# jczarnowski/DeepFactors

Measured on NVIDIA B200. Metric: keyframe-pair Jacobian+JtJ evals/sec (640x480, C=32), higher is better.
Workload: dtype f32

## Files before the change

### deepfactors_b200/csrc/dfk_api.cu

```cuda
#include <cuda_runtime.h>
#include <math.h>
#include <stdint.h>
#include <stdio.h>
#include <stdlib.h>
#include <string.h>

#include <algorithm>
#include <new>
#include <string>
#include <vector>

#include "dfk.h"
#include "dfk_internal.h"

using namespace dfk;

struct DfkContext {
  int device = 0;
  int num_sms = 1;
  int sm_limit = 0;
  cudaStream_t own_stream = nullptr;
  cudaStream_t stream = nullptr;
  std::string err;
  DfkSfmAlignerParams params;
// ... 6 lines not shown
  float* out_host = nullptr;
  float* code_dev = nullptr;
  float* track_dev = nullptr;
  size_t track_cap = 0;
  float* track_host = nullptr;
  size_t track_host_cap = 0;

  float* sparse_dev = nullptr;
  size_t sparse_cap = 0;
  float* sparse_host = nullptr;
  size_t sparse_host_cap = 0;
  SfmItemDev* items_dev = nullptr;
  size_t items_cap = 0;
  float* partials_dev = nullptr;
  size_t partials_cap = 0;
  struct RayTab {
    float fx, fy, u0, v0;
    uint32_t w, h;
    float* dev;
  };
  std::vector<RayTab> ray_cache;
  bool ray_miss = false;
  float* codes_dev = nullptr;
  size_t codes_cap = 0;
  std::vector<float> codes_host;
  float* records_dev = nullptr;
  size_t records_cap = 0;
  float* records_host = nullptr;
  size_t records_host_cap = 0;
  std::vector<SfmItemDev> items_host;
// ... 198 lines not shown
  return m % n == 0 ? 1 : m;
}

template <typename T>
cudaError_t ensure(T** ptr, size_t* cap, size_t need)
{
  if (*cap >= need) return cudaSuccess;
  const size_t old_cap = *cap;
  if (*ptr) cudaFree(*ptr);
  *ptr = nullptr;
  *cap = 0;
  size_t n = std::max(need, old_cap * 2);
  cudaError_t e = cudaMalloc(reinterpret_cast<void**>(ptr), n * sizeof(T));
  if (e == cudaSuccess) *cap = n;
  return e;
}

DfkStatus build_items(DfkHandle h, const DfkSfmWorkItem* items, int n, int code_size, int tile_px, int max_ctas,
                      bool want_ray_tabs, const float* codes_dev, SfmLaunchPlan* plan)
{
  h->ray_miss = false;
  const DfkDenseSfmParams& sp = h->params.sfmparams;
  h->items_host.resize(n);
  uint32_t tile_cursor = 0;
  for (int i = 0; i < n; ++i) {
    const DfkSfmWorkItem& w = items[i];
    SfmItemDev& d = h->items_host[i];
    const uint32_t W = w.img0.width, H = w.img0.height;
    if (W == 0 || H == 0) return fail(h, DFK_ERR_INVALID_ARG, "[SfmAligner::RunStep] empty image");
    if (!img_ok(&w.img0, W, H, 1) || !img_ok(&w.img1, W, H, 1) || !img_ok(&w.dpt0, W, H, 1) ||
// ... 168 lines not shown
                                cudaMemcpyHostToDevice, h->stream),
             "[SfmAligner::RunStep] code upload failed");
  const size_t pfloats = tc ? (size_t)kTcPartialFloats : sfm_partial_floats(code_size);
  DFK_CUDA(h, ensure(&h->items_dev, &h->items_cap, (size_t)n), "[SfmAligner::RunStep] scratch allocation failed");
  DFK_CUDA(h, ensure(&h->partials_dev, &h->partials_cap, (size_t)plan.num_partials * pfloats),
           "[SfmAligner::RunStep] scratch allocation failed");
  DFK_CUDA(h, cudaMemcpyAsync(h->items_dev, h->items_host.data(), sizeof(SfmItemDev) * n, cudaMemcpyHostToDevice,
                              h->stream),
           "[SfmAligner::RunStep] work list upload failed");
  cudaEvent_t ev0 = nullptr, ev1 = nullptr;
  if (h->profiling) {
    DfkStatus ps = profile_events(h, &ev0, &ev1);
    if (ps != DFK_OK) return ps;
  }
  if (tc) {
    DFK_CUDA(h, launch_sfm_tc(h->items_dev, plan, h->ray_miss, h->partials_dev, h->stream, ev0, ev1),
             "[SfmAligner::RunStep] kernel launch failed");
    if (h->ray_miss) h->launches += 1;
  } else if (wide) {
    DFK_CUDA(h, launch_sfm_wide(code_size, h->items_dev, plan, h->partials_dev, h->stream, ev0, ev1),
             "[SfmAligner::RunStep] kernel launch failed");
  } else {
    DFK_CUDA(h, launch_sfm_fp32(code_size, h->items_dev, plan, h->partials_dev, records_dev, h->stream, ev0, ev1),
             "[SfmAligner::RunStep] kernel launch failed");
  }
  DFK_CUDA(h, launch_sfm_finalize(code_size, tc, h->items_dev, n, h->partials_dev, records_dev, h->stream),
           "[SfmAligner::RunStep] kernel launch failed");
  h->launches += 2;
  return DFK_OK;
}

}

extern "C" {

int dfk_version(void) { return DFK_VERSION; }

const char* dfk_status_string(DfkStatus s)
{
  switch (s) {
    case DFK_OK: return "ok";
// ... 47 lines not shown
  } catch (...) {
    return DFK_ERR_NOMEM;
  }
}

DfkStatus dfk_destroy(DfkHandle h)
{
  try {
    if (!h) return DFK_OK;
    DeviceGuard guard(h->device);
    if (h->own_stream) cudaStreamSynchronize(h->own_stream);
    cudaFree(h->simple_scratch); cudaFree(h->counter); cudaFree(h->out_dev); cudaFree(h->code_dev);
    cudaFree(h->track_dev);
    cudaFree(h->codes_dev);
    if (h->track_host) cudaFreeHost(h->track_host);
    cudaFree(h->items_dev); cudaFree(h->partials_dev); cudaFree(h->records_dev);
    for (auto& r : h->ray_cache) cudaFree(r.dev);
    if (h->out_host) cudaFreeHost(h->out_host);
    if (h->records_host) cudaFreeHost(h->records_host);
    for (cudaEvent_t e : h->ev_pool) cudaEventDestroy(e);
    if (h->own_stream) cudaStreamDestroy(h->own_stream);
    delete h;
    return DFK_OK;
  } catch (...) {
    return oom(h);
  }
}

DfkStatus dfk_set_stream(DfkHandle h, void* cuda_stream)
{
  try {
// ... 952 lines not shown
```

### deepfactors_b200/csrc/dfk_internal.h

```cpp
#pragma once

#include <cuda_runtime.h>
#include <stdint.h>

#include <string>
#include <vector>

#include "dfk.h"

namespace dfk {

struct SfmItemDev {
  float q[4];
  float t[3];
  float R[9];
  float fx, fy, u0, v0;
  float border;
  float ulim;
  float vlim;
  float min_dpt, avg_dpt, huber_delta;
  const float* img0;
  const float* img1;
  const float* dpt0;
  float* valid0;
// ... 22 lines not shown
template <int C>
struct SfmCfg {
  static constexpr int NF = C + 7;
  static constexpr int NFP = (NF + 7) & ~7;
  static constexpr int NB = NFP / 8;
  static constexpr int NBLK = NB * (NB + 1) / 2;
  static constexpr int PARTIAL_FLOATS = NFP * NFP + 8;
};

constexpr int kTilePixels = 256;
constexpr int kTcTilePixels = 128;
constexpr int kTcRows = 80;
constexpr int kTcCols = 40;
constexpr int kTcRowsPad = 96;
constexpr int kTcPartialFloats = kTcRowsPad * kTcCols + 8;

struct SfmLaunchPlan {
  int num_items = 0;
  int num_tiles = 0;
  int num_ctas = 0;
  int num_partials = 0;
  int max_ctas_per_item = 0;
};

cudaError_t launch_sfm_fp32(int code_size, const SfmItemDev* items_dev, const SfmLaunchPlan& plan,
                            float* partials_dev, float* records_dev, cudaStream_t stream,
                            cudaEvent_t ev_start = nullptr, cudaEvent_t ev_stop = nullptr);
cudaError_t launch_sfm_finalize(int code_size, bool tc, const SfmItemDev* items_dev, int num_items,
                                const float* partials_dev, float* records_dev, cudaStream_t stream);
constexpr int sfm_wide_tile_pixels(int code_size) { return code_size >= 128 ? 64 : 128; }
bool sfm_wide_supported(int code_size);
cudaError_t launch_sfm_wide(int code_size, const SfmItemDev* items_dev, const SfmLaunchPlan& plan,
                            float* partials_dev, cudaStream_t stream, cudaEvent_t ev_start = nullptr,
                            cudaEvent_t ev_stop = nullptr);
bool sfm_tc_supported(int code_size);
cudaError_t launch_sfm_tc(const SfmItemDev* items_dev, const SfmLaunchPlan& plan, bool build_ray_tables,
                          float* partials_dev, cudaStream_t stream, cudaEvent_t ev_start = nullptr,
                          cudaEvent_t ev_stop = nullptr);
size_t sfm_partial_floats(int code_size);
constexpr int sfm_fp32_ctas_per_sm(int code_size) { return code_size <= 8 ? 2 : 1; }
bool sfm_fp32_supported(int code_size);
int sfm_max_ctas();

struct PixelCam {
  float q[4], t[3];
  float fx, fy, u0, v0, border, ulim, vlim, min_dpt;
};
struct View {
  const float* ptr;
  uint32_t pitch;
};
cudaError_t launch_se3_step(const PixelCam& pc, float huber_delta, int width, int height, View img0, View img1,
                            View dpt0, View grad1, bool grad_aligned, float* scratch, unsigned int* counter,
// ... 52 lines not shown
```

### deepfactors_b200/csrc/dfk_sfm_finalize.cu

```cuda
#include <cuda_runtime.h>
#include <stdint.h>

#include "dfk_internal.h"

namespace dfk {

namespace {

constexpr int kFinWarps = 8;
constexpr int kFinUnroll = 4;

__device__ __forceinline__ int packed_index(int i, int j, int NP) { return i * NP - (i * (i - 1)) / 2 + (j - i); }

__device__ __forceinline__ int tc_hrow(int f) { return f < 32 ? f : 64 + (f - 32); }
__device__ __forceinline__ int tc_lrow(int f) { return f < 32 ? 32 + f : 72 + (f - 32); }

template <int C, bool TC>
__global__ void __launch_bounds__(kFinWarps * 32)
sfm_finalize_kernel(const SfmItemDev* __restrict__ items, const float* __restrict__ partials,
                    float* __restrict__ records)
{
  using Cfg = SfmCfg<C>;
  constexpr int NFP = Cfg::NFP;
  constexpr int NP = 12 + C;
  constexpr int NH = NP * (NP + 1) / 2;
  constexpr int REC = NH + NP + 2;
  constexpr int NE = (C + 7 > 49) ? (C + 7) : 49;
  constexpr int EPL = (NE + 31) / 32;
  constexpr int PSTRIDE = TC ? kTcPartialFloats : Cfg::PARTIAL_FLOATS;
  constexpr int INL_OFF = TC ? kTcRowsPad * kTcCols : NFP * NFP;
  constexpr int NOFF = TC ? 3 : 1;
  __shared__ float red[kFinWarps][EPL * 32];
  __shared__ unsigned int red_inl[kFinWarps];
  __shared__ float sum[EPL * 32];

  cudaGridDependencySynchronize();
  const SfmItemDev& I = items[blockIdx.x];
  const int unit = blockIdx.y;
  const int warp = threadIdx.x >> 5, lane = threadIdx.x & 31;
  const float* P = partials + (size_t)I.partial_begin * PSTRIDE;
  const int np = (int)I.num_ctas;

  int off[EPL][NOFF];
  bool act[EPL];
#pragma unroll
  for (int q = 0; q < EPL; ++q) {
    const int e = q * 32 + lane;
    int fi, fj;
    if (unit < C) {
      act[q] = (unit + e) < (C + 7);
      fi = unit;
      fj = unit + e;
    } else {
      const int r = e / 7, c = e - 7 * r;
      act[q] = (e < 49) && (c >= r);
      fi = C + r;
      fj = C + c;
    }
    if (!act[q]) {
      fi = 0;
      fj = 0;
    }
    if constexpr (TC) {
      off[q][0] = fj * kTcRowsPad + tc_hrow(fi);
      off[q][1] = fj * kTcRowsPad + tc_lrow(fi);
      off[q][2] = fi * kTcRowsPad + tc_lrow(fj);
    } else {
      off[q][0] = fi * NFP + fj;
    }
  }
  float part[EPL];
#pragma unroll
  for (int q = 0; q < EPL; ++q) part[q] = 0.0f;
  unsigned int inl = 0;
  for (int k0 = warp; k0 < np; k0 += kFinWarps * kFinUnroll) {
    float v[kFinUnroll][EPL];
    unsigned int vi[kFinUnroll];
#pragma unroll
    for (int u = 0; u < kFinUnroll; ++u) {
      const int k = k0 + u * kFinWarps;
      const bool on = k < np;
      const float* Pk = P + (size_t)(on ? k : 0) * PSTRIDE;
#pragma unroll
      for (int q = 0; q < EPL; ++q) {
        v[u][q] = 0.0f;
        if (on && act[q]) {
          if constexpr (TC) v[u][q] = (Pk[off[q][0]] + Pk[off[q][1]]) + Pk[off[q][2]];
          else v[u][q] = Pk[off[q][0]];
        }
      }
      vi[u] = (on && unit == C && lane == 0) ? reinterpret_cast<const unsigned int*>(Pk)[INL_OFF] : 0u;
    }
#pragma unroll
    for (int u = 0; u < kFinUnroll; ++u) {
#pragma unroll
      for (int q = 0; q < EPL; ++q) part[q] += v[u][q];
      inl += vi[u];
    }
  }
#pragma unroll
  for (int q = 0; q < EPL; ++q) red[warp][q * 32 + lane] = part[q];
  if (lane == 0) red_inl[warp] = inl;
  __syncthreads();
  if (warp == 0) {
#pragma unroll
    for (int q = 0; q < EPL; ++q) {
      float s = 0.0f;
#pragma unroll
      for (int w = 0; w < kFinWarps; ++w) s += red[w][q * 32 + lane];
      sum[q * 32 + lane] = s;
    }
  }
  __syncthreads();

  float* rec = records + (size_t)blockIdx.x * REC;
  float* JtJ = rec;
  float* Jtr = rec + NH;
  if (unit < C) {
    const int c = unit;
    for (int e = threadIdx.x; e < C - c; e += blockDim.x) JtJ[packed_index(12 + c, 12 + c + e, NP)] = sum[e];
    if (threadIdx.x < 12) {
      const int j = threadIdx.x % 6;
      const float* Pm = threadIdx.x < 6 ? I.P0 : I.P1;
      float s = 0.0f;
#pragma unroll
      for (int k = 0; k < 6; ++k) s = fmaf(Pm[k * 6 + j], sum[(C - c) + k], s);
      JtJ[packed_index(threadIdx.x, 12 + c, NP)] = s;
    }
    if (threadIdx.x == 12) Jtr[12 + c] = sum[(C - c) + 6];
  } else {
    __shared__ float Gaa[6][6];
    __shared__ float T0[6][6];
    __shared__ float T1[6][6];
    if (threadIdx.x < 36) {
      const int r = threadIdx.x / 6, c = threadIdx.x % 6;
      Gaa[r][c] = (c >= r) ? sum[r * 7 + c] : sum[c * 7 + r];
    }
    __syncthreads();
    if (threadIdx.x < 72) {
      const int m = threadIdx.x / 36, r = (threadIdx.x % 36) / 6, c = threadIdx.x % 6;
      const float* Pm = m ? I.P1 : I.P0;
      float s = 0.0f;
#pragma unroll
      for (int k = 0; k < 6; ++k) s = fmaf(Gaa[r][k], Pm[k * 6 + c], s);
      (m ? T1 : T0)[r][c] = s;
    }
    __syncthreads();
    for (int e = threadIdx.x; e < 144; e += blockDim.x) {
      const int i = e / 12, j = e % 12;
      if (j < i) continue;
      const float* Pa = (i < 6) ? I.P0 : I.P1;
      const float(*Tb)[6] = (j < 6) ? T0 : T1;
      const int ii = i % 6, jj = j % 6;
      float s = 0.0f;
#pragma unroll
      for (int k = 0; k < 6; ++k) s = fmaf(Pa[k * 6 + ii], Tb[k][jj], s);
      JtJ[packed_index(i, j, NP)] = s;
    }
    if (threadIdx.x >= 160 && threadIdx.x < 172) {
      const int i = threadIdx.x - 160;
      const float* Pa = (i < 6) ? I.P0 : I.P1;
      float s = 0.0f;
#pragma unroll
      for (int k = 0; k < 6; ++k) s = fmaf(Pa[k * 6 + (i % 6)], sum[k * 7 + 6], s);
      Jtr[i] = s;
    }
    if (threadIdx.x == 192) {
      unsigned int tot = 0;
      for (int w = 0; w < kFinWarps; ++w) tot += red_inl[w];
      rec[NH + NP] = sum[48];
      reinterpret_cast<unsigned int*>(rec)[NH + NP + 1] = tot;
    }
  }
}

template <int C, bool TC>
cudaError_t launch_fin(const SfmItemDev* items_dev, int num_items, const float* partials_dev, float* records_dev,
                       cudaStream_t stream)
{
  cudaLaunchConfig_t cfg{};
  cfg.gridDim = dim3(num_items, C + 1);
  cfg.blockDim = dim3(kFinWarps * 32);
  cfg.dynamicSmemBytes = 0;
  cfg.stream = stream;
  cudaLaunchAttribute attr[1];
  attr[0].id = cudaLaunchAttributeProgrammaticStreamSerialization;
  attr[0].val.programmaticStreamSerializationAllowed = 1;
  cfg.attrs = attr;
  cfg.numAttrs = 1;
  return cudaLaunchKernelEx(&cfg, sfm_finalize_kernel<C, TC>, items_dev, partials_dev, records_dev);
}

}

cudaError_t launch_sfm_finalize(int code_size, bool tc, const SfmItemDev* items_dev, int num_items,
                                const float* partials_dev, float* records_dev, cudaStream_t stream)
{
  if (tc) {
    if (code_size != 32) return cudaErrorInvalidValue;
    return launch_fin<32, true>(items_dev, num_items, partials_dev, records_dev, stream);
  }
  switch (code_size) {
    case 8: return launch_fin<8, false>(items_dev, num_items, partials_dev, records_dev, stream);
    case 16: return launch_fin<16, false>(items_dev, num_items, partials_dev, records_dev, stream);
    case 32: return launch_fin<32, false>(items_dev, num_items, partials_dev, records_dev, stream);
    case 64: return launch_fin<64, false>(items_dev, num_items, partials_dev, records_dev, stream);
    case 128: return launch_fin<128, false>(items_dev, num_items, partials_dev, records_dev, stream);
    default: return cudaErrorInvalidValue;
  }
}

}
```

### deepfactors_b200/csrc/dfk_sfm_tc.cu

```cuda
#include <cuda_runtime.h>
#include <stdint.h>
#include <stdio.h>
#include <stdlib.h>

#include "dfk_async.cuh"
#include "dfk_geom.cuh"
#include "dfk_internal.h"
#include "dfk_tcgen05.cuh"

namespace dfk {

namespace {

constexpr int C = 32;
constexpr int TILE = kTcTilePixels;
constexpr int NFE = 12;
constexpr int THREADS = 512;
#ifndef DFK_TC_SLOTS
#define DFK_TC_SLOTS 7
#endif
constexpr int NSLOT = DFK_TC_SLOTS;
constexpr uint32_t ATOM_BYTES = 512;
constexpr uint32_t MN_STRIDE = 8 * ATOM_BYTES;
constexpr uint32_t SLOT_BYTES = 3 * MN_STRIDE;
// ... 39 lines not shown
  uint32_t img0_pitch, img1_pitch, dpt0_pitch, valid0_pitch, jac_pitch, grad1_pitch, dpt_out_pitch;
  uint32_t width, height, num_pixels, tile_begin, num_tiles, perm_mul, flags, slot, mag_tiles, mag_width;
  alignas(16) float code[C];
};

struct Smem {
  alignas(1024) unsigned char op[NSLOT][SLOT_BYTES];
  alignas(128) ItemSmem item[NFE];
  alignas(8) uint64_t full[NSLOT];
  uint64_t done[NFE];
  uint64_t d_full[2];
  uint64_t d_empty[2];
  alignas(16) SlotMeta meta[NSLOT];
  alignas(16) ChainRec chain[2];
  uint32_t tmem_base;
};
static_assert(sizeof(ItemSmem) * NFE >= MN_STRIDE, "the ring's tail pad");

__device__ __forceinline__ void load_item(ItemSmem& dst, const SfmItemDev& src, int lane, int cta)
{
  if (lane < 4) dst.q[lane] = src.q[lane];
  if (lane >= 4 && lane < 7) dst.t[lane - 4] = src.t[lane - 4];
  if (lane >= 8 && lane < 17) dst.R[lane - 8] = src.R[lane - 8];
  if (lane == 17) {
    dst.fx = src.fx; dst.fy = src.fy; dst.u0 = src.u0; dst.v0 = src.v0;
    dst.border = src.border; dst.ulim = src.ulim; dst.vlim = src.vlim;
    dst.min_dpt = src.min_dpt; dst.avg_dpt = src.avg_dpt; dst.huber_delta = src.huber_delta;
  }
  if (lane == 18) {
    dst.img0 = src.img0; dst.img1 = src.img1; dst.dpt0 = src.dpt0; dst.valid0 = src.valid0;
// ... 14 lines not shown
  }
  if (src.flags & ITEM_FLAG_FUSED_DEPTH) dst.code[lane] = __ldg(src.code + lane);
}

__device__ __forceinline__ uint32_t div_magic(uint32_t a, uint32_t b, uint32_t mag, uint32_t& rem)
{
  uint32_t q = __umulhi(a, mag);
  uint32_t r = a - q * b;
  if (r >= b) {
    ++q;
    r -= b;
  }
  rem = r;
  return q;
}
__device__ __forceinline__ float tf32_trunc(float v) { return __uint_as_float(__float_as_uint(v) & 0xffffe000u); }

#ifdef DFK_TC_WATCHDOG
__device__ __noinline__ void wd_wait(uint64_t* bar, uint32_t parity, int what, int idx)
{
  for (long long spin = 0; spin < 2000000; ++spin)
    if (mbar_try_wait(bar, parity)) return;
  if ((threadIdx.x & 31) == 0)
    printf("[dfk tc watchdog] cta %d warp %d stuck: wait %d index %d parity %u\n", (int)blockIdx.x, (int)(threadIdx.x >> 5), what,
           idx, parity);
  __trap();
}
#define TC_WAIT(bar, parity, what, idx) wd_wait(bar, parity, what, idx)
#else
#define TC_WAIT(bar, parity, what, idx) mbar_wait(bar, parity)
#endif

__device__ __forceinline__ void sts128(uint32_t addr, float a, float b, float c, float d)
{
  asm volatile("st.shared.v4.f32 [%0], {%1, %2, %3, %4};" ::"r"(addr), "f"(a), "f"(b), "f"(c), "f"(d));
}

__device__ __forceinline__ float4 load_chunk(const float* __restrict__ p, bool aligned16)
{
  if (aligned16) return __ldg(reinterpret_cast<const float4*>(p));
  return make_float4(__ldg(p), __ldg(p + 1), __ldg(p + 2), __ldg(p + 3));
}

__global__ void __launch_bounds__(THREADS, 2)
sfm_step_tc_kernel(const SfmItemDev* __restrict__ items, int num_items, int num_tiles, float* __restrict__ partials)
{
  extern __shared__ unsigned char smem_raw[];
  Smem& sm = *reinterpret_cast<Smem*>(smem_raw + ((1024u - (smem_u32(smem_raw) & 1023u)) & 1023u));
  const int tid = threadIdx.x;
  const int warp = tid >> 5;
  const int lane = tid & 31;
  const int cta = blockIdx.x;
  const int G = gridDim.x;
  const int g_lo = (int)(((long long)cta * num_tiles) / G);
  const int g_hi = (int)(((long long)(cta + 1) * num_tiles) / G);
  const int ntiles = g_hi - g_lo;
  const int nblocks = 4 * ntiles;
  (void)num_items;

  if (tid == 0) {
    for (int s = 0; s < NSLOT; ++s) {
      mbar_init(&sm.full[s], 1);
    }
    for (int w = 0; w < NFE; ++w) mbar_init(&sm.done[w], 1);
    for (int b = 0; b < 2; ++b) {
      mbar_init(&sm.d_full[b], 2);
      mbar_init(&sm.d_empty[b], 3);
    }
    mbar_fence_init();
  }
  for (int e = tid; e < (int)(NSLOT * SLOT_BYTES / 16); e += THREADS)
    reinterpret_cast<float4*>(&sm.op[0][0])[e] = make_float4(0.f, 0.f, 0.f, 0.f);
  if (warp == 15) {
// ... 15 lines not shown
  if (ntiles > 0) {
    if (warp < NFE) {
      ItemSmem& I = sm.item[warp];
      int it = 0;
      int cur_item = -1;
      uint32_t item_lo = 0, item_hi = 0;
      uint32_t done_phase = 0;
      for (int j = warp; j < nblocks; j += NFE) {
        const int i = j >> 2, b = j & 3;
        const int g = g_lo + i;
        if (cur_item < 0 || (uint32_t)g >= item_hi) {
          while ((uint32_t)g >= items[it].tile_begin + items[it].num_tiles) ++it;
          __syncwarp();
          load_item(I, items[it], lane, cta);
          __syncwarp();
          cur_item = it;
          item_lo = I.tile_begin;
          item_hi = I.tile_begin + I.num_tiles;
        }
        const bool seq_changed = (b == 0) && ((i == 0) || ((uint32_t)(g - 1) < item_lo));
        const uint32_t k = (uint32_t)g - item_lo;
        uint32_t tau;
        div_magic(k * I.perm_mul, I.num_tiles, I.mag_tiles, tau);
        const uint32_t p0 = tau * TILE;
        const uint32_t n = min((uint32_t)TILE, I.num_pixels - p0);
        const uint32_t s = 32u * (uint32_t)b + (uint32_t)lane;
        const bool inb = s < n;
        const bool blk_live = 32u * (uint32_t)b < n;
        const uint32_t W = I.width;
        const bool a16 = (I.flags & ITEM_FLAG_BULK) != 0;
// ... 249 lines not shown
                if (c < ncol) __stcg(dcol + c * kTcRowsPad, __uint_as_float(v[c]));
            } else {
#pragma unroll
              for (int c = 0; c < 16; ++c)
                if (c < ncol)
                  asm volatile("red.global.add.f32 [%0], %1;" ::"l"(dcol + c * kTcRowsPad), "f"(__uint_as_float(v[c])) : "memory");
            }
          }
        }
        tc_fence_before();
        __syncwarp();
        if (lane == 0) mbar_arrive(&sm.d_empty[b]);
        if (rec.item_end && ow == 0 && lane == 0) reinterpret_cast<unsigned int*>(P)[kTcRowsPad * kTcCols] = rec.inliers;
        if (rec.last) break;
      }
    }
  }

  tc_fence_before();
  __syncthreads();
  if (warp == 15) tmem_dealloc(tbase, TMEM_COLS);
}

}

__global__ void sfm_ray_tables_kernel(const SfmItemDev* __restrict__ items, float* __restrict__ tabs)
{
  (void)tabs;
  const SfmItemDev& I = items[blockIdx.x];
  float* dst = const_cast<float*>(I.ray_tab);
  for (uint32_t x = threadIdx.x; x < I.width; x += blockDim.x) dst[x] = ray_coord((float)x, I.u0, I.fx);
  for (uint32_t y = threadIdx.x; y < I.height; y += blockDim.x) dst[I.width + y] = ray_coord((float)y, I.v0, I.fy);
}

bool sfm_tc_supported(int code_size) { return code_size == 32; }

size_t sfm_tc_smem_bytes() { return sizeof(Smem) + 1024; }

cudaError_t launch_sfm_tc(const SfmItemDev* items_dev, const SfmLaunchPlan& plan, bool build_ray_tables,
                          float* partials_dev, cudaStream_t stream, cudaEvent_t ev_start, cudaEvent_t ev_stop)
{
  const size_t smem = sizeof(Smem) + 1024;
  static const cudaError_t attr_err =
      cudaFuncSetAttribute(sfm_step_tc_kernel, cudaFuncAttributeMaxDynamicSharedMemorySize, (int)(sizeof(Smem) + 1024));
  cudaError_t err = attr_err;
  if (err != cudaSuccess) return err;
  if (build_ray_tables) {
    sfm_ray_tables_kernel<<<plan.num_items, 256, 0, stream>>>(items_dev, nullptr);
    err = cudaGetLastError();
    if (err != cudaSuccess) return err;
  }
  if (ev_start) cudaEventRecord(ev_start, stream);
  sfm_step_tc_kernel<<<plan.num_ctas, THREADS, smem, stream>>>(items_dev, plan.num_items, plan.num_tiles, partials_dev);
  if (ev_stop) cudaEventRecord(ev_stop, stream);
  return cudaGetLastError();
}

}
```

### deepfactors_b200/csrc/dfk_window.cu

```cuda
#include <cuda_runtime.h>
#include <stdint.h>

#include "dfk_internal.h"

namespace dfk {

namespace {

__device__ __forceinline__ int packed_index(int i, int j, int NP) { return i * NP - (i * (i - 1)) / 2 + (j - i); }
__device__ __forceinline__ float rec_h(const float* rec, int a, int b, int NP)
{
  return a <= b ? rec[packed_index(a, b, NP)] : rec[packed_index(b, a, NP)];
}

__global__ void __launch_bounds__(256)
window_assemble_kernel(WindowDev w, const float* __restrict__ records, float* __restrict__ out)
{
  const int C = w.code_size, B = 6 + C, NP = 12 + C;
  const int NH = NP * (NP + 1) / 2, REC = NH + NP + 2;
  const int job = blockIdx.x;
  if (job < w.num_keyframes) {
    const int k = job;
    float* D = out + (size_t)k * B * B;
    float* g = out + (size_t)w.num_keyframes * B * B + (size_t)k * B;
    const int a0 = w.kf0_ptr[k], a1 = w.kf0_ptr[k + 1];
    const int b0 = w.kf1_ptr[k], b1 = w.kf1_ptr[k + 1];
    for (int e = threadIdx.x; e < B * B + B; e += blockDim.x) {
      float s = 0.0f;
      if (e < B * B) {
        const int r = e / B, c = e - r * B;
        const int lr = r < 6 ? r : 6 + r, lc = c < 6 ? c : 6 + c;
        for (int q = a0; q < a1; ++q) s += rec_h(records + (size_t)w.kf0_items[q] * REC, lr, lc, NP);
        if (r < 6 && c < 6)
          for (int q = b0; q < b1; ++q) s += rec_h(records + (size_t)w.kf1_items[q] * REC, 6 + r, 6 + c, NP);
        D[e] = s;
      } else {
        const int r = e - B * B;
        const int lr = r < 6 ? r : 6 + r;
        for (int q = a0; q < a1; ++q) s -= records[(size_t)w.kf0_items[q] * REC + NH + lr];
        if (r < 6)
          for (int q = b0; q < b1; ++q) s -= records[(size_t)w.kf1_items[q] * REC + NH + 6 + r];
        g[r] = s;
      }
    }
  } else if (job < w.num_keyframes + w.num_pairs) {
    const int p = job - w.num_keyframes;
    float* O = out + (size_t)w.num_keyframes * (B * B + B) + (size_t)p * B * 6;
    const int i0 = w.pair_ptr[p], i1 = w.pair_ptr[p + 1];
    for (int e = threadIdx.x; e < B * 6; e += blockDim.x) {
      const int r = e / 6, c = e - r * 6;
      const int lr = r < 6 ? r : 6 + r;
      float s = 0.0f;
      for (int q = i0; q < i1; ++q) s += rec_h(records + (size_t)w.pair_items[q] * REC, lr, 6 + c, NP);
      O[e] = s;
    }
  } else {
    __shared__ float red_f[8], red_i[8];
    float f = 0.0f, ni = 0.0f;
    for (int i = threadIdx.x; i < w.num_items; i += blockDim.x) {
      const float* rec = records + (size_t)i * REC;
      const uint32_t inl = __float_as_uint(rec[NH + NP + 1]);
      if (inl > 0) f += rec[NH + NP] / (float)inl * w.item_area[i];
      ni += (float)inl;
    }
    for (int o = 16; o > 0; o >>= 1) {
      f += __shfl_xor_sync(0xffffffffu, f, o);
      ni += __shfl_xor_sync(0xffffffffu, ni, o);
    }
    if ((threadIdx.x & 31) == 0) {
      red_f[threadIdx.x >> 5] = f;
      red_i[threadIdx.x >> 5] = ni;
    }
    __syncthreads();
    if (threadIdx.x == 0) {
      float sf = 0.0f, si = 0.0f;
      for (int k = 0; k < (int)(blockDim.x >> 5); ++k) {
        sf += red_f[k];
        si += red_i[k];
      }
      float* tail = out + (size_t)w.num_keyframes * (B * B + B) + (size_t)w.num_pairs * B * 6;
      tail[0] = sf;
      tail[1] = si;
    }
  }
}

}

cudaError_t launch_window_assemble(const WindowDev& w, const float* records_dev, float* out_dev, cudaStream_t stream)
{
  window_assemble_kernel<<<w.num_keyframes + w.num_pairs + 1, 256, 0, stream>>>(w, records_dev, out_dev);
  return cudaGetLastError();
}

}
```

Before: 46610.

## Fuse TC finalize into main kernel via ticketed chain reductions; flatten window assembly

The tensor-core SfM kernel now reduces its own per-CTA partials. Each CTA takes a ticket, and the last arrivers sum partials into up to eight chain buffers. The final chain collector then expands the Gram into the packed JtJ/Jtr record, so the separate finalize launch is removed for the TC path. The window assembly kernel is also reworked to one thread per output element with programmatic dependent launch. This trades a launch and a pass over partials for atomics, threadfences and zeroed ticket scratch.

```diff
diff --git a/deepfactors_b200/csrc/dfk_api.cu b/deepfactors_b200/csrc/dfk_api.cu
--- a/deepfactors_b200/csrc/dfk_api.cu
+++ b/deepfactors_b200/csrc/dfk_api.cu
@@ -44,6 +44,10 @@
   size_t items_cap = 0;
   float* partials_dev = nullptr;
   size_t partials_cap = 0;
+  unsigned int* tickets_dev = nullptr;
+  size_t tickets_cap = 0;
+  float* chains_dev = nullptr;
+  size_t chains_cap = 0;
   struct RayTab {
     float fx, fy, u0, v0;
     uint32_t w, h;
@@ -272,6 +276,14 @@
   cudaError_t e = cudaMalloc(reinterpret_cast<void**>(ptr), n * sizeof(T));
   if (e == cudaSuccess) *cap = n;
   return e;
+}
+
+cudaError_t ensure_zeroed(unsigned int** ptr, size_t* cap, size_t need, cudaStream_t stream)
+{
+  if (*cap >= need) return cudaSuccess;
+  cudaError_t e = ensure(ptr, cap, need);
+  if (e != cudaSuccess) return e;
+  return cudaMemsetAsync(*ptr, 0, *cap * sizeof(unsigned int), stream);
 }
 
 DfkStatus build_items(DfkHandle h, const DfkSfmWorkItem* items, int n, int code_size, int tile_px, int max_ctas,
@@ -470,9 +482,16 @@
     if (ps != DFK_OK) return ps;
   }
   if (tc) {
-    DFK_CUDA(h, launch_sfm_tc(h->items_dev, plan, h->ray_miss, h->partials_dev, h->stream, ev0, ev1),
+    DFK_CUDA(h, ensure_zeroed(&h->tickets_dev, &h->tickets_cap, (size_t)n * (kTcChains + 1), h->stream),
+             "[SfmAligner::RunStep] scratch allocation failed");
+    DFK_CUDA(h, ensure(&h->chains_dev, &h->chains_cap, (size_t)n * kTcChains * kTcChainFloats),
+             "[SfmAligner::RunStep] scratch allocation failed");
+    DFK_CUDA(h, launch_sfm_tc(h->items_dev, plan, h->ray_miss, h->partials_dev, h->tickets_dev, h->chains_dev,
+                              records_dev, h->stream, ev0, ev1),
              "[SfmAligner::RunStep] kernel launch failed");
     if (h->ray_miss) h->launches += 1;
+    h->launches += 1;
+    return DFK_OK;
   } else if (wide) {
     DFK_CUDA(h, launch_sfm_wide(code_size, h->items_dev, plan, h->partials_dev, h->stream, ev0, ev1),
              "[SfmAligner::RunStep] kernel launch failed");
@@ -480,7 +499,7 @@
     DFK_CUDA(h, launch_sfm_fp32(code_size, h->items_dev, plan, h->partials_dev, records_dev, h->stream, ev0, ev1),
              "[SfmAligner::RunStep] kernel launch failed");
   }
-  DFK_CUDA(h, launch_sfm_finalize(code_size, tc, h->items_dev, n, h->partials_dev, records_dev, h->stream),
+  DFK_CUDA(h, launch_sfm_finalize(code_size, h->items_dev, n, h->partials_dev, records_dev, h->stream),
            "[SfmAligner::RunStep] kernel launch failed");
   h->launches += 2;
   return DFK_OK;
@@ -558,7 +577,7 @@
     cudaFree(h->track_dev);
     cudaFree(h->codes_dev);
     if (h->track_host) cudaFreeHost(h->track_host);
-    cudaFree(h->items_dev); cudaFree(h->partials_dev); cudaFree(h->records_dev);
+    cudaFree(h->items_dev); cudaFree(h->partials_dev); cudaFree(h->tickets_dev); cudaFree(h->chains_dev); cudaFree(h->records_dev);
     for (auto& r : h->ray_cache) cudaFree(r.dev);
     if (h->out_host) cudaFreeHost(h->out_host);
     if (h->records_host) cudaFreeHost(h->records_host);
diff --git a/deepfactors_b200/csrc/dfk_internal.h b/deepfactors_b200/csrc/dfk_internal.h
--- a/deepfactors_b200/csrc/dfk_internal.h
+++ b/deepfactors_b200/csrc/dfk_internal.h
@@ -60,6 +60,8 @@
 constexpr int kTcCols = 40;
 constexpr int kTcRowsPad = 96;
 constexpr int kTcPartialFloats = kTcRowsPad * kTcCols + 8;
+constexpr int kTcChains = 8;
+constexpr int kTcChainFloats = 804;
 
 struct SfmLaunchPlan {
   int num_items = 0;
@@ -72,8 +74,8 @@
 cudaError_t launch_sfm_fp32(int code_size, const SfmItemDev* items_dev, const SfmLaunchPlan& plan,
                             float* partials_dev, float* records_dev, cudaStream_t stream,
                             cudaEvent_t ev_start = nullptr, cudaEvent_t ev_stop = nullptr);
-cudaError_t launch_sfm_finalize(int code_size, bool tc, const SfmItemDev* items_dev, int num_items,
-                                const float* partials_dev, float* records_dev, cudaStream_t stream);
+cudaError_t launch_sfm_finalize(int code_size, const SfmItemDev* items_dev, int num_items, const float* partials_dev,
+                                float* records_dev, cudaStream_t stream);
 constexpr int sfm_wide_tile_pixels(int code_size) { return code_size >= 128 ? 64 : 128; }
 bool sfm_wide_supported(int code_size);
 cudaError_t launch_sfm_wide(int code_size, const SfmItemDev* items_dev, const SfmLaunchPlan& plan,
@@ -81,8 +83,8 @@
                             cudaEvent_t ev_stop = nullptr);
 bool sfm_tc_supported(int code_size);
 cudaError_t launch_sfm_tc(const SfmItemDev* items_dev, const SfmLaunchPlan& plan, bool build_ray_tables,
-                          float* partials_dev, cudaStream_t stream, cudaEvent_t ev_start = nullptr,
-                          cudaEvent_t ev_stop = nullptr);
+                          float* partials_dev, unsigned int* tickets_dev, float* chains_dev, float* records_dev,
+                          cudaStream_t stream, cudaEvent_t ev_start = nullptr, cudaEvent_t ev_stop = nullptr);
 size_t sfm_partial_floats(int code_size);
 constexpr int sfm_fp32_ctas_per_sm(int code_size) { return code_size <= 8 ? 2 : 1; }
 bool sfm_fp32_supported(int code_size);
diff --git a/deepfactors_b200/csrc/dfk_sfm_expand.cuh b/deepfactors_b200/csrc/dfk_sfm_expand.cuh
--- /dev/null
+++ b/deepfactors_b200/csrc/dfk_sfm_expand.cuh
@@ -0,0 +1,125 @@
+#pragma once
+
+#include <cuda_runtime.h>
+#include <stdint.h>
+
+namespace dfk {
+
+__device__ __forceinline__ int rec_packed_index(int i, int j, int NP) { return i * NP - (i * (i - 1)) / 2 + (j - i); }
+
+template <int C>
+__device__ __forceinline__ bool gram_unit_entry(int unit, int e, int& fi, int& fj)
+{
+  bool act;
+  if (unit < C) {
+    act = (unit + e) < (C + 7);
+    fi = unit;
+    fj = unit + e;
+  } else {
+    const int r = e / 7, c = e - 7 * r;
+    act = (e < 49) && (c >= r);
+    fi = C + r;
+    fj = C + c;
+  }
+  if (!act) {
+    fi = 0;
+    fj = 0;
+  }
+  return act;
+}
+
+template <int C>
+__host__ __device__ constexpr int gram_unit_offset(int u)
+{
+  return u * (C + 7) - (u * (u - 1)) / 2;
+}
+template <int C>
+__host__ __device__ constexpr int gram_flat_floats()
+{
+  return gram_unit_offset<C>(C) + 49;
+}
+
+template <int C>
+__device__ __forceinline__ void gram_flat_unit(int f, int& unit, int& e)
+{
+  unit = 0;
+  while (unit < C && f >= C + 7 - unit) {
+    f -= C + 7 - unit;
+    ++unit;
+  }
+  e = f;
+}
+
+template <int C>
+__device__ __forceinline__ void expand_code_row(int c, int t, const float* g, const float* P0, const float* P1,
+                                                float* rec)
+{
+  constexpr int NP = 12 + C;
+  constexpr int NH = NP * (NP + 1) / 2;
+  float* JtJ = rec;
+  float* Jtr = rec + NH;
+  if (t < C - c) {
+    JtJ[rec_packed_index(12 + c, 12 + c + t, NP)] = g[t];
+  } else if (t < C - c + 12) {
+    const int i = t - (C - c);
+    const int j = i % 6;
+    const float* Pm = i < 6 ? P0 : P1;
+    float s = 0.0f;
+#pragma unroll
+    for (int k = 0; k < 6; ++k) s = fmaf(Pm[k * 6 + j], g[(C - c) + k], s);
+    JtJ[rec_packed_index(i, 12 + c, NP)] = s;
+  } else if (t == C - c + 12) {
+    Jtr[12 + c] = g[(C - c) + 6];
+  }
+}
+
+__device__ __forceinline__ void expand_pose_gaa(int t, const float* g, float (*Gaa)[6])
+{
+  if (t < 36) {
+    const int r = t / 6, c = t % 6;
+    Gaa[r][c] = (c >= r) ? g[r * 7 + c] : g[c * 7 + r];
+  }
+}
+__device__ __forceinline__ void expand_pose_t(int t, const float (*Gaa)[6], const float* P0, const float* P1,
+                                              float (*T0)[6], float (*T1)[6])
+{
+  if (t < 72) {
+    const int m = t / 36, r = (t % 36) / 6, c = t % 6;
+    const float* Pm = m ? P1 : P0;
+    float s = 0.0f;
+#pragma unroll
+    for (int k = 0; k < 6; ++k) s = fmaf(Gaa[r][k], Pm[k * 6 + c], s);
+    (m ? T1 : T0)[r][c] = s;
+  }
+}
+template <int C>
+__device__ __forceinline__ void expand_pose_out(int t, const float* g, const float* P0, const float* P1,
+                                                const float (*T0)[6], const float (*T1)[6], unsigned int inliers,
+                                                float* rec)
+{
+  constexpr int NP = 12 + C;
+  constexpr int NH = NP * (NP + 1) / 2;
+  if (t < 144) {
+    const int i = t / 12, j = t % 12;
+    if (j < i) return;
+    const float* Pa = (i < 6) ? P0 : P1;
+    const float(*Tb)[6] = (j < 6) ? T0 : T1;
+    const int ii = i % 6, jj = j % 6;
+    float s = 0.0f;
+#pragma unroll
+    for (int k = 0; k < 6; ++k) s = fmaf(Pa[k * 6 + ii], Tb[k][jj], s);
+    rec[rec_packed_index(i, j, NP)] = s;
+  } else if (t < 156) {
+    const int i = t - 144;
+    const float* Pa = (i < 6) ? P0 : P1;
+    float s = 0.0f;
+#pragma unroll
+    for (int k = 0; k < 6; ++k) s = fmaf(Pa[k * 6 + (i % 6)], g[k * 7 + 6], s);
+    rec[NH + i] = s;
+  } else if (t == 156) {
+    rec[NH + NP] = g[48];
+    reinterpret_cast<unsigned int*>(rec)[NH + NP + 1] = inliers;
+  }
+}
+
+}
diff --git a/deepfactors_b200/csrc/dfk_sfm_finalize.cu b/deepfactors_b200/csrc/dfk_sfm_finalize.cu
--- a/deepfactors_b200/csrc/dfk_sfm_finalize.cu
+++ b/deepfactors_b200/csrc/dfk_sfm_finalize.cu
@@ -2,6 +2,7 @@
 #include <stdint.h>
 
 #include "dfk_internal.h"
+#include "dfk_sfm_expand.cuh"
 
 namespace dfk {
 
@@ -10,12 +11,7 @@
 constexpr int kFinWarps = 8;
 constexpr int kFinUnroll = 4;
 
-__device__ __forceinline__ int packed_index(int i, int j, int NP) { return i * NP - (i * (i - 1)) / 2 + (j - i); }
-
-__device__ __forceinline__ int tc_hrow(int f) { return f < 32 ? f : 64 + (f - 32); }
-__device__ __forceinline__ int tc_lrow(int f) { return f < 32 ? 32 + f : 72 + (f - 32); }
-
-template <int C, bool TC>
+template <int C>
 __global__ void __launch_bounds__(kFinWarps * 32)
 sfm_finalize_kernel(const SfmItemDev* __restrict__ items, const float* __restrict__ partials,
                     float* __restrict__ records)
@@ -23,13 +19,11 @@
   using Cfg = SfmCfg<C>;
   constexpr int NFP = Cfg::NFP;
   constexpr int NP = 12 + C;
-  constexpr int NH = NP * (NP + 1) / 2;
-  constexpr int REC = NH + NP + 2;
+  constexpr int REC = (NP * (NP + 1)) / 2 + NP + 2;
   constexpr int NE = (C + 7 > 49) ? (C + 7) : 49;
   constexpr int EPL = (NE + 31) / 32;
-  constexpr int PSTRIDE = TC ? kTcPartialFloats : Cfg::PARTIAL_FLOATS;
-  constexpr int INL_OFF = TC ? kTcRowsPad * kTcCols : NFP * NFP;
-  constexpr int NOFF = TC ? 3 : 1;
+  constexpr int PSTRIDE = Cfg::PARTIAL_FLOATS;
+  constexpr int INL_OFF = NFP * NFP;
   __shared__ float red[kFinWarps][EPL * 32];
   __shared__ unsigned int red_inl[kFinWarps];
   __shared__ float sum[EPL * 32];
@@ -41,33 +35,13 @@
   const float* P = partials + (size_t)I.partial_begin * PSTRIDE;
   const int np = (int)I.num_ctas;
 
-  int off[EPL][NOFF];
+  int off[EPL];
   bool act[EPL];
 #pragma unroll
   for (int q = 0; q < EPL; ++q) {
-    const int e = q * 32 + lane;
     int fi, fj;
-    if (unit < C) {
-      act[q] = (unit + e) < (C + 7);
-      fi = unit;
-      fj = unit + e;
-    } else {
-      const int r = e / 7, c = e - 7 * r;
-      act[q] = (e < 49) && (c >= r);
-      fi = C + r;
-      fj = C + c;
-    }
-    if (!act[q]) {
-      fi = 0;
-      fj = 0;
-    }
-    if constexpr (TC) {
-      off[q][0] = fj * kTcRowsPad + tc_hrow(fi);
-      off[q][1] = fj * kTcRowsPad + tc_lrow(fi);
-      off[q][2] = fi * kTcRowsPad + tc_lrow(fj);
-    } else {
-      off[q][0] = fi * NFP + fj;
-    }
+    act[q] = gram_unit_entry<C>(unit, q * 32 + lane, fi, fj);
+    off[q] = fi * NFP + fj;
   }
   float part[EPL];
 #pragma unroll
@@ -82,13 +56,7 @@
       const bool on = k < np;
       const float* Pk = P + (size_t)(on ? k : 0) * PSTRIDE;
 #pragma unroll
-      for (int q = 0; q < EPL; ++q) {
-        v[u][q] = 0.0f;
-        if (on && act[q]) {
-          if constexpr (TC) v[u][q] = (Pk[off[q][0]] + Pk[off[q][1]]) + Pk[off[q][2]];
-          else v[u][q] = Pk[off[q][0]];
-        }
-      }
+      for (int q = 0; q < EPL; ++q) v[u][q] = (on && act[q]) ? Pk[off[q]] : 0.0f;
       vi[u] = (on && unit == C && lane == 0) ? reinterpret_cast<const unsigned int*>(Pk)[INL_OFF] : 0u;
     }
 #pragma unroll
@@ -114,67 +82,23 @@
   __syncthreads();
 
   float* rec = records + (size_t)blockIdx.x * REC;
-  float* JtJ = rec;
-  float* Jtr = rec + NH;
   if (unit < C) {
-    const int c = unit;
-    for (int e = threadIdx.x; e < C - c; e += blockDim.x) JtJ[packed_index(12 + c, 12 + c + e, NP)] = sum[e];
-    if (threadIdx.x < 12) {
-      const int j = threadIdx.x % 6;
-      const float* Pm = threadIdx.x < 6 ? I.P0 : I.P1;
-      float s = 0.0f;
-#pragma unroll
-      for (int k = 0; k < 6; ++k) s = fmaf(Pm[k * 6 + j], sum[(C - c) + k], s);
-      JtJ[packed_index(threadIdx.x, 12 + c, NP)] = s;
-    }
-    if (threadIdx.x == 12) Jtr[12 + c] = sum[(C - c) + 6];
+    for (int t = threadIdx.x; t < C - unit + 13; t += blockDim.x) expand_code_row<C>(unit, t, sum, I.P0, I.P1, rec);
   } else {
     __shared__ float Gaa[6][6];
     __shared__ float T0[6][6];
     __shared__ float T1[6][6];
-    if (threadIdx.x < 36) {
-      const int r = threadIdx.x / 6, c = threadIdx.x % 6;
-      Gaa[r][c] = (c >= r) ? sum[r * 7 + c] : sum[c * 7 + r];
-    }
+    expand_pose_gaa(threadIdx.x, sum, Gaa);
     __syncthreads();
-    if (threadIdx.x < 72) {
-      const int m = threadIdx.x / 36, r = (threadIdx.x % 36) / 6, c = threadIdx.x % 6;
-      const float* Pm = m ? I.P1 : I.P0;
-      float s = 0.0f;
-#pragma unroll
-      for (int k = 0; k < 6; ++k) s = fmaf(Gaa[r][k], Pm[k * 6 + c], s);
-      (m ? T1 : T0)[r][c] = s;
-    }
+    expand_pose_t(threadIdx.x, Gaa, I.P0, I.P1, T0, T1);
     __syncthreads();
-    for (int e = threadIdx.x; e < 144; e += blockDim.x) {
-      const int i = e / 12, j = e % 12;
-      if (j < i) continue;
-      const float* Pa = (i < 6) ? I.P0 : I.P1;
-      const float(*Tb)[6] = (j < 6) ? T0 : T1;
-      const int ii = i % 6, jj = j % 6;
-      float s = 0.0f;
-#pragma unroll
-      for (int k = 0; k < 6; ++k) s = fmaf(Pa[k * 6 + ii], Tb[k][jj], s);
-      JtJ[packed_index(i, j, NP)] = s;
-    }
-    if (threadIdx.x >= 160 && threadIdx.x < 172) {
-      const int i = threadIdx.x - 160;
-      const float* Pa = (i < 6) ? I.P0 : I.P1;
-      float s = 0.0f;
-#pragma unroll
-      for (int k = 0; k < 6; ++k) s = fmaf(Pa[k * 6 + (i % 6)], sum[k * 7 + 6], s);
-      Jtr[i] = s;
-    }
-    if (threadIdx.x == 192) {
-      unsigned int tot = 0;
-      for (int w = 0; w < kFinWarps; ++w) tot += red_inl[w];
-      rec[NH + NP] = sum[48];
-      reinterpret_cast<unsigned int*>(rec)[NH + NP + 1] = tot;
-    }
+    unsigned int tot = 0;
+    for (int w = 0; w < kFinWarps; ++w) tot += red_inl[w];
+    expand_pose_out<C>(threadIdx.x, sum, I.P0, I.P1, T0, T1, tot, rec);
   }
 }
 
-template <int C, bool TC>
+template <int C>
 cudaError_t launch_fin(const SfmItemDev* items_dev, int num_items, const float* partials_dev, float* records_dev,
                        cudaStream_t stream)
 {
@@ -188,24 +112,20 @@
   attr[0].val.programmaticStreamSerializationAllowed = 1;
   cfg.attrs = attr;
   cfg.numAttrs = 1;
-  return cudaLaunchKernelEx(&cfg, sfm_finalize_kernel<C, TC>, items_dev, partials_dev, records_dev);
+  return cudaLaunchKernelEx(&cfg, sfm_finalize_kernel<C>, items_dev, partials_dev, records_dev);
 }
 
 }
 
-cudaError_t launch_sfm_finalize(int code_size, bool tc, const SfmItemDev* items_dev, int num_items,
-                                const float* partials_dev, float* records_dev, cudaStream_t stream)
+cudaError_t launch_sfm_finalize(int code_size, const SfmItemDev* items_dev, int num_items, const float* partials_dev,
+                                float* records_dev, cudaStream_t stream)
 {
-  if (tc) {
-    if (code_size != 32) return cudaErrorInvalidValue;
-    return launch_fin<32, true>(items_dev, num_items, partials_dev, records_dev, stream);
-  }
   switch (code_size) {
-    case 8: return launch_fin<8, false>(items_dev, num_items, partials_dev, records_dev, stream);
-    case 16: return launch_fin<16, false>(items_dev, num_items, partials_dev, records_dev, stream);
-    case 32: return launch_fin<32, false>(items_dev, num_items, partials_dev, records_dev, stream);
-    case 64: return launch_fin<64, false>(items_dev, num_items, partials_dev, records_dev, stream);
-    case 128: return launch_fin<128, false>(items_dev, num_items, partials_dev, records_dev, stream);
+    case 8: return launch_fin<8>(items_dev, num_items, partials_dev, records_dev, stream);
+    case 16: return launch_fin<16>(items_dev, num_items, partials_dev, records_dev, stream);
+    case 32: return launch_fin<32>(items_dev, num_items, partials_dev, records_dev, stream);
+    case 64: return launch_fin<64>(items_dev, num_items, partials_dev, records_dev, stream);
+    case 128: return launch_fin<128>(items_dev, num_items, partials_dev, records_dev, stream);
     default: return cudaErrorInvalidValue;
   }
 }
diff --git a/deepfactors_b200/csrc/dfk_sfm_tc.cu b/deepfactors_b200/csrc/dfk_sfm_tc.cu
--- a/deepfactors_b200/csrc/dfk_sfm_tc.cu
+++ b/deepfactors_b200/csrc/dfk_sfm_tc.cu
@@ -6,6 +6,7 @@
 #include "dfk_async.cuh"
 #include "dfk_geom.cuh"
 #include "dfk_internal.h"
+#include "dfk_sfm_expand.cuh"
 #include "dfk_tcgen05.cuh"
 
 namespace dfk {
@@ -77,6 +78,7 @@
   alignas(16) SlotMeta meta[NSLOT];
   alignas(16) ChainRec chain[2];
   uint32_t tmem_base;
+  int first_item;
 };
 static_assert(sizeof(ItemSmem) * NFE >= MN_STRIDE, "the ring's tail pad");
 
@@ -121,6 +123,38 @@
   rem = r;
   return q;
 }
+__device__ __forceinline__ int tc_hrow(int f) { return f < 32 ? f : 64 + (f - 32); }
+__device__ __forceinline__ int tc_lrow(int f) { return f < 32 ? 32 + f : 72 + (f - 32); }
+
+constexpr int EPI_THREADS = NFE * 32;
+constexpr int EPI_BAR = 1;
+constexpr int GRAM = gram_flat_floats<C>();
+constexpr int GRAM_PAD = (GRAM + 3) & ~3;
+constexpr int REC = (12 + C) * (13 + C) / 2 + (12 + C) + 2;
+static_assert(GRAM + 1 <= kTcChainFloats, "chain partial: the Gram + the inliers");
+static_assert((GRAM_PAD + 3 * 36 + 1) * 4 <= NSLOT * SLOT_BYTES, "epilogue scratch lives in the operand ring");
+
+__device__ __forceinline__ void epi_sync() { asm volatile("bar.sync %0, %1;" ::"n"(EPI_BAR), "n"(EPI_THREADS) : "memory"); }
+__device__ __forceinline__ bool epi_any(bool p)
+{
+  uint32_t r;
+  asm volatile(
+      "{\n\t.reg .pred p, q;\n\tsetp.ne.u32 p, %1, 0;\n\tbar.red.or.pred q, %2, %3, p;\n\tselp.u32 %0, 1, 0, q;\n\t}"
+      : "=r"(r)
+      : "r"((uint32_t)p), "n"(EPI_BAR), "n"(EPI_THREADS)
+      : "memory");
+  return r != 0;
+}
+__device__ __forceinline__ bool ticket_last(unsigned int* t, unsigned int want)
+{
+  unsigned int old;
+  asm volatile("atom.acq_rel.gpu.global.add.u32 %0, [%1], 1;" : "=r"(old) : "l"(t) : "memory");
+  __threadfence();
+  const bool last = old + 1u == want;
+  if (last) *t = 0u;
+  return last;
+}
+
 __device__ __forceinline__ float tf32_trunc(float v) { return __uint_as_float(__float_as_uint(v) & 0xffffe000u); }
 
 #ifdef DFK_TC_WATCHDOG
@@ -150,7 +184,8 @@
 }
 
 __global__ void __launch_bounds__(THREADS, 2)
-sfm_step_tc_kernel(const SfmItemDev* __restrict__ items, int num_items, int num_tiles, float* __restrict__ partials)
+sfm_step_tc_kernel(const SfmItemDev* __restrict__ items, int num_items, int num_tiles, float* __restrict__ partials,
+                   unsigned int* __restrict__ tickets, float* __restrict__ chains, float* __restrict__ records)
 {
   extern __shared__ unsigned char smem_raw[];
   Smem& sm = *reinterpret_cast<Smem*>(smem_raw + ((1024u - (smem_u32(smem_raw) & 1023u)) & 1023u));
@@ -163,7 +198,6 @@
   const int g_hi = (int)(((long long)(cta + 1) * num_tiles) / G);
   const int ntiles = g_hi - g_lo;
   const int nblocks = 4 * ntiles;
-  (void)num_items;
 
   if (tid == 0) {
     for (int s = 0; s < NSLOT; ++s) {
@@ -209,6 +243,7 @@
           __syncwarp();
           load_item(I, items[it], lane, cta);
           __syncwarp();
+          if (j == 0 && lane == 0) sm.first_item = it;
           cur_item = it;
           item_lo = I.tile_begin;
           item_hi = I.tile_begin + I.num_tiles;
@@ -488,12 +523,96 @@
         if (rec.item_end && ow == 0 && lane == 0) reinterpret_cast<unsigned int*>(P)[kTcRowsPad * kTcCols] = rec.inliers;
         if (rec.last) break;
       }
+      __threadfence();
     }
   }
 
   tc_fence_before();
   __syncthreads();
   if (warp == 15) tmem_dealloc(tbase, TMEM_COLS);
+
+  if (warp < NFE && ntiles > 0) {
+    float* g = reinterpret_cast<float*>(&sm.op[0][0]);
+    float(*Gaa)[6] = reinterpret_cast<float(*)[6]>(g + GRAM_PAD);
+    float(*T0)[6] = Gaa + 6;
+    float(*T1)[6] = Gaa + 12;
+    unsigned int* inl_s = reinterpret_cast<unsigned int*>(g + GRAM_PAD + 3 * 36);
+    for (int it = sm.first_item; it < num_items; ++it) {
+      const SfmItemDev& I = items[it];
+      if (I.tile_begin >= (uint32_t)g_hi) break;
+      const int nc = (int)I.num_ctas;
+      const int w = (cta - (int)I.first_cta) % kTcChains;
+      unsigned int* tk = tickets + (size_t)it * (kTcChains + 1);
+      if (!epi_any(tid == 0 && ticket_last(tk + w, (unsigned)((nc - w + kTcChains - 1) / kTcChains)))) continue;
+
+      const float* P = partials + (size_t)I.partial_begin * kTcPartialFloats;
+      float* chain = chains + ((size_t)it * kTcChains + w) * kTcChainFloats;
+      for (int f = tid; f < GRAM; f += EPI_THREADS) {
+        int unit, e, fi, fj;
+        gram_flat_unit<C>(f, unit, e);
+        float s = 0.0f;
+        if (gram_unit_entry<C>(unit, e, fi, fj)) {
+          const int o0 = fj * kTcRowsPad + tc_hrow(fi);
+          const int o1 = fj * kTcRowsPad + tc_lrow(fi);
+          const int o2 = fi * kTcRowsPad + tc_lrow(fj);
+          int k = w;
+          for (; k + 3 * kTcChains < nc; k += 4 * kTcChains) {
+            float v[4];
+#pragma unroll
+            for (int u = 0; u < 4; ++u) {
+              const float* Pk = P + (size_t)(k + u * kTcChains) * kTcPartialFloats;
+              v[u] = (__ldcg(Pk + o0) + __ldcg(Pk + o1)) + __ldcg(Pk + o2);
+            }
+#pragma unroll
+            for (int u = 0; u < 4; ++u) s += v[u];
+          }
+          for (; k < nc; k += kTcChains) {
+            const float* Pk = P + (size_t)k * kTcPartialFloats;
+            s += (__ldcg(Pk + o0) + __ldcg(Pk + o1)) + __ldcg(Pk + o2);
+          }
+        }
+        __stcg(chain + f, s);
+      }
+      if (tid == 0) {
+        unsigned int inl = 0;
+        for (int k = w; k < nc; k += kTcChains)
+          inl += __ldcg(reinterpret_cast<const unsigned int*>(P + (size_t)k * kTcPartialFloats) + kTcRowsPad * kTcCols);
+        __stcg(reinterpret_cast<unsigned int*>(chain) + GRAM, inl);
+      }
+      __threadfence();
+      epi_sync();
+      if (!epi_any(tid == 0 && ticket_last(tk + kTcChains, (unsigned)min(nc, kTcChains)))) continue;
+
+      const int nch = min(nc, kTcChains);
+      const float* ch = chains + (size_t)it * kTcChains * kTcChainFloats;
+      for (int f = tid; f < GRAM; f += EPI_THREADS) {
+        float v[kTcChains];
+#pragma unroll
+        for (int c = 0; c < kTcChains; ++c) v[c] = c < nch ? __ldcg(ch + (size_t)c * kTcChainFloats + f) : 0.0f;
+        float s = 0.0f;
+#pragma unroll
+        for (int c = 0; c < kTcChains; ++c) s += v[c];
+        g[f] = s;
+      }
+      if (tid == 0) {
+        unsigned int inl = 0;
+        for (int c = 0; c < nch; ++c) inl += __ldcg(reinterpret_cast<const unsigned int*>(ch + (size_t)c * kTcChainFloats) + GRAM);
+        *inl_s = inl;
+      }
+      epi_sync();
+      float* rec = records + (size_t)it * REC;
+      for (int t = tid; t < C * (C + 13); t += EPI_THREADS) {
+        const int c = t / (C + 13), e = t - c * (C + 13);
+        expand_code_row<C>(c, e, g + gram_unit_offset<C>(c), I.P0, I.P1, rec);
+      }
+      const float* gp = g + gram_unit_offset<C>(C);
+      expand_pose_gaa(tid, gp, Gaa);
+      epi_sync();
+      expand_pose_t(tid, Gaa, I.P0, I.P1, T0, T1);
+      epi_sync();
+      expand_pose_out<C>(tid, gp, I.P0, I.P1, T0, T1, *inl_s, rec);
+    }
+  }
 }
 
 }
@@ -512,7 +631,8 @@
 size_t sfm_tc_smem_bytes() { return sizeof(Smem) + 1024; }
 
 cudaError_t launch_sfm_tc(const SfmItemDev* items_dev, const SfmLaunchPlan& plan, bool build_ray_tables,
-                          float* partials_dev, cudaStream_t stream, cudaEvent_t ev_start, cudaEvent_t ev_stop)
+                          float* partials_dev, unsigned int* tickets_dev, float* chains_dev, float* records_dev,
+                          cudaStream_t stream, cudaEvent_t ev_start, cudaEvent_t ev_stop)
 {
   const size_t smem = sizeof(Smem) + 1024;
   static const cudaError_t attr_err =
@@ -525,7 +645,8 @@
     if (err != cudaSuccess) return err;
   }
   if (ev_start) cudaEventRecord(ev_start, stream);
-  sfm_step_tc_kernel<<<plan.num_ctas, THREADS, smem, stream>>>(items_dev, plan.num_items, plan.num_tiles, partials_dev);
+  sfm_step_tc_kernel<<<plan.num_ctas, THREADS, smem, stream>>>(items_dev, plan.num_items, plan.num_tiles, partials_dev,
+                                                               tickets_dev, chains_dev, records_dev);
   if (ev_stop) cudaEventRecord(ev_stop, stream);
   return cudaGetLastError();
 }
diff --git a/deepfactors_b200/csrc/dfk_window.cu b/deepfactors_b200/csrc/dfk_window.cu
--- a/deepfactors_b200/csrc/dfk_window.cu
+++ b/deepfactors_b200/csrc/dfk_window.cu
@@ -7,55 +7,51 @@
 
 namespace {
 
+constexpr int kAsmThreads = 256;
+
 __device__ __forceinline__ int packed_index(int i, int j, int NP) { return i * NP - (i * (i - 1)) / 2 + (j - i); }
 __device__ __forceinline__ float rec_h(const float* rec, int a, int b, int NP)
 {
   return a <= b ? rec[packed_index(a, b, NP)] : rec[packed_index(b, a, NP)];
 }
 
-__global__ void __launch_bounds__(256)
+__global__ void __launch_bounds__(kAsmThreads)
 window_assemble_kernel(WindowDev w, const float* __restrict__ records, float* __restrict__ out)
 {
   const int C = w.code_size, B = 6 + C, NP = 12 + C;
   const int NH = NP * (NP + 1) / 2, REC = NH + NP + 2;
-  const int job = blockIdx.x;
-  if (job < w.num_keyframes) {
-    const int k = job;
-    float* D = out + (size_t)k * B * B;
-    float* g = out + (size_t)w.num_keyframes * B * B + (size_t)k * B;
-    const int a0 = w.kf0_ptr[k], a1 = w.kf0_ptr[k + 1];
-    const int b0 = w.kf1_ptr[k], b1 = w.kf1_ptr[k + 1];
-    for (int e = threadIdx.x; e < B * B + B; e += blockDim.x) {
-      float s = 0.0f;
-      if (e < B * B) {
-        const int r = e / B, c = e - r * B;
-        const int lr = r < 6 ? r : 6 + r, lc = c < 6 ? c : 6 + c;
-        for (int q = a0; q < a1; ++q) s += rec_h(records + (size_t)w.kf0_items[q] * REC, lr, lc, NP);
-        if (r < 6 && c < 6)
-          for (int q = b0; q < b1; ++q) s += rec_h(records + (size_t)w.kf1_items[q] * REC, 6 + r, 6 + c, NP);
-        D[e] = s;
-      } else {
-        const int r = e - B * B;
-        const int lr = r < 6 ? r : 6 + r;
-        for (int q = a0; q < a1; ++q) s -= records[(size_t)w.kf0_items[q] * REC + NH + lr];
-        if (r < 6)
-          for (int q = b0; q < b1; ++q) s -= records[(size_t)w.kf1_items[q] * REC + NH + 6 + r];
-        g[r] = s;
-      }
-    }
-  } else if (job < w.num_keyframes + w.num_pairs) {
-    const int p = job - w.num_keyframes;
-    float* O = out + (size_t)w.num_keyframes * (B * B + B) + (size_t)p * B * 6;
-    const int i0 = w.pair_ptr[p], i1 = w.pair_ptr[p + 1];
-    for (int e = threadIdx.x; e < B * 6; e += blockDim.x) {
+  const int K = w.num_keyframes;
+  const int n_diag = K * B * B, n_grad = K * B, n_pair = w.num_pairs * B * 6;
+  const int n_elem = n_diag + n_grad + n_pair;
+  const int nb_elem = (n_elem + kAsmThreads - 1) / kAsmThreads;
+  cudaGridDependencySynchronize();
+  if ((int)blockIdx.x < nb_elem) {
+    const int o = blockIdx.x * kAsmThreads + threadIdx.x;
+    if (o >= n_elem) return;
+    float s = 0.0f;
+    if (o < n_diag) {
+      const int k = o / (B * B), e = o - k * (B * B);
+      const int r = e / B, c = e - r * B;
+      const int lr = r < 6 ? r : 6 + r, lc = c < 6 ? c : 6 + c;
+      for (int q = w.kf0_ptr[k]; q < w.kf0_ptr[k + 1]; ++q) s += rec_h(records + (size_t)w.kf0_items[q] * REC, lr, lc, NP);
+      if (r < 6 && c < 6)
+        for (int q = w.kf1_ptr[k]; q < w.kf1_ptr[k + 1]; ++q)
+          s += rec_h(records + (size_t)w.kf1_items[q] * REC, 6 + r, 6 + c, NP);
+    } else if (o < n_diag + n_grad) {
+      const int k = (o - n_diag) / B, r = (o - n_diag) - k * B;
+      const int lr = r < 6 ? r : 6 + r;
+      for (int q = w.kf0_ptr[k]; q < w.kf0_ptr[k + 1]; ++q) s -= records[(size_t)w.kf0_items[q] * REC + NH + lr];
+      if (r < 6)
+        for (int q = w.kf1_ptr[k]; q < w.kf1_ptr[k + 1]; ++q) s -= records[(size_t)w.kf1_items[q] * REC + NH + 6 + r];
+    } else {
+      const int p = (o - n_diag - n_grad) / (B * 6), e = (o - n_diag - n_grad) - p * (B * 6);
       const int r = e / 6, c = e - r * 6;
       const int lr = r < 6 ? r : 6 + r;
-      float s = 0.0f;
-      for (int q = i0; q < i1; ++q) s += rec_h(records + (size_t)w.pair_items[q] * REC, lr, 6 + c, NP);
-      O[e] = s;
+      for (int q = w.pair_ptr[p]; q < w.pair_ptr[p + 1]; ++q) s += rec_h(records + (size_t)w.pair_items[q] * REC, lr, 6 + c, NP);
     }
+    out[o] = s;
   } else {
-    __shared__ float red_f[8], red_i[8];
+    __shared__ float red_f[kAsmThreads / 32], red_i[kAsmThreads / 32];
     float f = 0.0f, ni = 0.0f;
     for (int i = threadIdx.x; i < w.num_items; i += blockDim.x) {
       const float* rec = records + (size_t)i * REC;
@@ -78,9 +74,8 @@
         sf += red_f[k];
         si += red_i[k];
       }
-      float* tail = out + (size_t)w.num_keyframes * (B * B + B) + (size_t)w.num_pairs * B * 6;
-      tail[0] = sf;
-      tail[1] = si;
+      out[n_elem] = sf;
+      out[n_elem + 1] = si;
     }
   }
 }
@@ -89,8 +84,20 @@
 
 cudaError_t launch_window_assemble(const WindowDev& w, const float* records_dev, float* out_dev, cudaStream_t stream)
 {
-  window_assemble_kernel<<<w.num_keyframes + w.num_pairs + 1, 256, 0, stream>>>(w, records_dev, out_dev);
-  return cudaGetLastError();
+  const int B = 6 + w.code_size;
+  const long long n_elem = (long long)w.num_keyframes * (B * B + B) + (long long)w.num_pairs * B * 6;
+  if (n_elem >= (1ll << 31) - kAsmThreads) return cudaErrorInvalidValue;
+  cudaLaunchConfig_t cfg{};
+  cfg.gridDim = dim3((unsigned)((n_elem + kAsmThreads - 1) / kAsmThreads) + 1);
+  cfg.blockDim = dim3(kAsmThreads);
+  cfg.dynamicSmemBytes = 0;
+  cfg.stream = stream;
+  cudaLaunchAttribute attr[1];
+  attr[0].id = cudaLaunchAttributeProgrammaticStreamSerialization;
+  attr[0].val.programmaticStreamSerializationAllowed = 1;
+  cfg.attrs = attr;
+  cfg.numAttrs = 1;
+  return cudaLaunchKernelEx(&cfg, window_assemble_kernel, w, records_dev, out_dev);
 }
 
 }
```

Measured after the change: 45090 (median of 6 runs). 3.3% lower.
